# qwang-sj/qwen3-asr.cpp

Hardware: AMD Instinct MI355X
Metric: RTFx (audio-sec/wall-sec) + decode tokens/sec, Qwen3-ASR-0.6B f16 (higher is better)
Workload: dtype f16

## Files before the change

qwen3-asr.cpp_amd/csrc/attention.hip:

```cpp
#include <algorithm>
#include <type_traits>
#include <cstdlib>
#include <stdexcept>

#include "dev_common.h"
#include "fx_chain.h"
#include "fx_decode.h"
#include "kernels.h"

namespace qasr {

#define EKS 66
#define EVS 68

__global__ __launch_bounds__(256) void enc_attn_kernel(const float *__restrict__ qkv, const int *__restrict__ seg_start,
                                                       const int *__restrict__ seg_len, int D, uint16_t *__restrict__ out,
                                                       float *__restrict__ out32) {
    __shared__ __attribute__((aligned(16))) float Ks[64 * EKS];
    __shared__ __attribute__((aligned(16))) float Vs[64 * EVS];
    const int b = blockIdx.z, h = blockIdx.y;
    const int N = seg_len[b], r0 = seg_start[b];
    const int qblk = blockIdx.x * 64;
    if (qblk >= N) return;
    const int tid = threadIdx.x, lane = tid & 63, wid = tid >> 6;
// ... 1009 lines not shown
        if (c0 + 128 < nkv) kvc_issue(kc, vc, c0 + 128, kcap, want_v, A, a.kv_nt);
        kvc_step(a, qa, knew, vnew, c0 + 64, pos, B, st, sdst);
    }
    if constexpr (FX) {
        __syncthreads();
        mark(2);
        decode_attn_exact_body(a, 2 * g + (wid >> 1), b, wid & 1, fxs + (wid >> 1) * a.max_ctx);
        if (a.trace) __syncthreads();
        mark(3);
        stamp_end(a.stamp);
        return;
    }
    if (sdst) { stamp_end(a.stamp); return; }
#pragma unroll
    for (int e = 0; e < 8; e++) {
        st.o0[e] += __shfl_xor(st.o0[e], 16, 64);
        st.o0[e] += __shfl_xor(st.o0[e], 32, 64);
        st.o1[e] += __shfl_xor(st.o1[e], 16, 64);
        st.o1[e] += __shfl_xor(st.o1[e], 32, 64);
    }
    if (sub == 0) {
        *(floatx4 *)&wo[wid][0][dl] = floatx4{st.o0[0], st.o0[1], st.o0[2], st.o0[3]};
        *(floatx4 *)&wo[wid][0][dl + 4] = floatx4{st.o0[4], st.o0[5], st.o0[6], st.o0[7]};
        *(floatx4 *)&wo[wid][1][dl] = floatx4{st.o1[0], st.o1[1], st.o1[2], st.o1[3]};
        *(floatx4 *)&wo[wid][1][dl + 4] = floatx4{st.o1[4], st.o1[5], st.o1[6], st.o1[7]};
    }
    if (lane == 0) {
        wst[wid][0][0] = st.m0; wst[wid][0][1] = st.l0;
        wst[wid][1][0] = st.m1; wst[wid][1][1] = st.l1;
    }
    __syncthreads();
    const int hh = tid >> 7, d = tid & 127;
    float M = -INFINITY;
#pragma unroll
    for (int w = 0; w < 4; w++) M = fmaxf(M, wst[w][hh][0]);
    float L = 0.f, O = 0.f;
#pragma unroll
    for (int w = 0; w < 4; w++) {
        const float mw = wst[w][hh][0];
        const float f = mw == -INFINITY ? 0.f : expf(mw - M);
        L = fmaf(wst[w][hh][1], f, L);
        O = fmaf(wo[w][hh][d], f, O);
    }
    const float inv = L > 0.f ? 1.0f / L : 0.f;
    const float v = O * inv;
    const long e = (long)b * QD + (2 * g + hh) * 128 + d;
    if (a.outq) {
        float am = fabsf(v);
#pragma unroll
        for (int o = 1; o < 32; o <<= 1) am = fmaxf(am, __shfl_xor(am, o, 64));
        a.outq[e] = q8_quant(v, am);
        if ((d & 31) == 0) a.outd[e >> 5] = q8_scale(am);
    } else if (a.out32) a.out32[e] = v;
    else a.out[e] = f_to_u16(v);
    stamp_end(a.stamp);
}

int decode_stream_slots() {
    int nb = 0, dev = 0, cus = 0;
    if (hipGetDevice(&dev) != hipSuccess || hipDeviceGetAttribute(&cus, hipDeviceAttributeMultiprocessorCount, dev) != hipSuccess ||
        hipOccupancyMaxActiveBlocksPerMultiprocessor(&nb, reinterpret_cast<const void *>(decode_attn_seq_kernel<0>), 256, 0) !=
            hipSuccess)
        return 0;
    return nb * cus;
}

constexpr int ORPW = 1, OPROJ_ROWS = 4 * ORPW;
__device__ __forceinline__ void oproj1_body(const GemvArgs o, const DecodeAttnArgs a, int j) {
    constexpr int K = 2048, NT = 4;
    const int lane = threadIdx.x & 63, wid = threadIdx.x >> 6;
    const int row0 = j * OPROJ_ROWS + wid * ORPW;
    for (int i = 0; i < a.oproj_delay; i++) __builtin_amdgcn_s_sleep(8);
    half8 wv[ORPW][NT];
#pragma unroll
    for (int r = 0; r < ORPW; r++)
#pragma unroll
        for (int t = 0; t < NT; t++)
            wv[r][t] = __builtin_nontemporal_load((const half8 *)(o.W + (long)(row0 + r) * K + t * 512 + lane * 8));
    __shared__ int oready;
    if (threadIdx.x == 0) {
        int ok = 0;
        for (int it = 0; it < a.poll_limit; it++) {
            if (__hip_atomic_load(a.att_done + (j & 7) * 16, __ATOMIC_RELAXED, __HIP_MEMORY_SCOPE_AGENT) >=
                (unsigned)a.n_kv_head) {
                ok = 1;
                break;
            }
            __builtin_amdgcn_s_sleep(4);
        }
        if (a.fence) {
            __builtin_amdgcn_fence(__ATOMIC_ACQUIRE, "agent");
            asm volatile("s_waitcnt vmcnt(0)" ::: "memory");
        }
        if (!ok) __hip_atomic_fetch_or(a.err, (unsigned)DEVERR_O_WAIT, __ATOMIC_RELAXED, __HIP_MEMORY_SCOPE_AGENT);
        oready = ok;
    }
    __syncthreads();
    if (!oready) return;
    u32x4 xv[NT];
    ld_sc1_x4_4(o.xh + lane * 8, xv);
    float res[ORPW];
#pragma unroll
    for (int r = 0; r < ORPW; r++)
        res[r] = __uint_as_float(__hip_atomic_load((const uint32_t *)(o.res + row0 + r), __ATOMIC_RELAXED, __HIP_MEMORY_SCOPE_AGENT));
#pragma unroll
    for (int r = 0; r < ORPW; r++) {
        float acc = 0.f;
#pragma unroll
        for (int t = 0; t < NT; t++) {
            const half8 h = __builtin_bit_cast(half8, xv[t]);
#pragma unroll
            for (int e = 0; e < 8; e++) acc = fmaf((float)wv[r][t][e], (float)h[e], acc);
        }
        acc = wave_sum(acc);
        if (lane == 0) o.out_f32[row0 + r] = fadd_rn(acc, res[r]);
    }
}

__device__ __forceinline__ void ld_sc1_x4_8(const void *base, const uint32_t *off, u32x4 *v) {
    asm volatile(
        "global_load_dwordx4 %0, %8, %16 sc1\n\t"
        "global_load_dwordx4 %1, %9, %16 sc1\n\t"
        "global_load_dwordx4 %2, %10, %16 sc1\n\t"
        "global_load_dwordx4 %3, %11, %16 sc1\n\t"
        "global_load_dwordx4 %4, %12, %16 sc1\n\t"
        "global_load_dwordx4 %5, %13, %16 sc1\n\t"
        "global_load_dwordx4 %6, %14, %16 sc1\n\t"
        "global_load_dwordx4 %7, %15, %16 sc1\n\t"
        "s_waitcnt vmcnt(0)"
        : "=&v"(v[0]), "=&v"(v[1]), "=&v"(v[2]), "=&v"(v[3]), "=&v"(v[4]), "=&v"(v[5]), "=&v"(v[6]), "=&v"(v[7])
        : "v"(off[0]), "v"(off[1]), "v"(off[2]), "v"(off[3]), "v"(off[4]), "v"(off[5]), "v"(off[6]), "v"(off[7]), "s"(base)
        : "memory");
}
__host__ __device__ inline int fx_chain_wgs(int fx, int n_kv_head) { return fx ? n_kv_head : 0; }
struct alignas(16) ChainLds {
    float fsc[2][DX_KC / DX_B * FX_ST];
    uint16_t kmask[2][DX_KC / 16];
    float fwl[2];
};
__device__ __forceinline__ float fx1_gather_weights(const DecodeAttnArgs &a, const int g, const int n, ChainLds &C, const int trow) {
    auto &fsc = C.fsc;
    const int tid = threadIdx.x, lane = tid & 63, wid = tid >> 6;
    const int hh = wid >> 1, wu = __builtin_amdgcn_readfirstlane(wid & 1);
    auto mark = [&](int slot) {
        if (a.trace && tid == 0) a.trace[(long)trow * 8 + slot] = rt_now();
    };
    const uint32_t tag = gran_tag(a.pos[0], a.layer);
    const int np = (n + 1) >> 1;
    {
        const int ld = sgran_ld(a.max_ctx);
        const unsigned long long *gb = a.sgran + (long)(2 * g) * ld;
        uint32_t go[DX_KC / 256];
#pragma unroll
        for (int u = 0; u < DX_KC / 256; u++) {
            const int q = tid + 256 * (u >> 1);
            go[u] = q < np ? (uint32_t)(((u & 1) * ld + 2 * q) * 8) : 0u;
        }
        u32x4 gv[DX_KC / 256];
        bool ok = false;
        int it = 0;
        unsigned long long tis = 0;
        for (; it < a.poll_limit; it++) {
            if (a.trace) tis = rt_now();
            ld_sc1_x4_8(gb, go, gv);
            ok = true;
#pragma unroll
            for (int u = 0; u < DX_KC / 256; u++) {
                const int q = tid + 256 * (u >> 1);
                if (q < np) ok = ok && gv[u][1] == tag && (2 * q + 1 >= n || gv[u][3] == tag);
            }
            if (__syncthreads_and(ok)) break;
            __builtin_amdgcn_s_sleep(2);
        }
        if (a.trace && tid == 0) {
            a.trace[(4010L + g) * 8 + 5] = (unsigned long long)it + 1;
            a.trace[(4010L + g) * 8 + 6] = tis;
        }
        if (!ok && tid == 0) __hip_atomic_fetch_or(a.err, (unsigned)DEVERR_SCORE_WAIT, __ATOMIC_RELAXED, __HIP_MEMORY_SCOPE_AGENT);
#pragma unroll
        for (int u = 0; u < DX_KC / 256; u++) {
            const int q = tid + 256 * (u >> 1), j = 2 * q;
            if (q < np)
                *(float2 *)&fsc[u & 1][(j >> 5) * FX_ST + (j & 31)] = make_float2(__uint_as_float(gv[u][0]), __uint_as_float(gv[u][2]));
        }
    }
    __syncthreads();
    mark(2);
    auto &fwl = C.fwl;
    auto &kmask = C.kmask;
    float M, S;
    {
        float *row = fsc[hh] + lane * FX_ST;
        float sv[DX_B];
#pragma unroll
        for (int i = 0; i < DX_B; i += 4) {
            const floatx4 r = *(const floatx4 *)&row[i];
#pragma unroll
            for (int e = 0; e < 4; e++) sv[i + e] = lane * DX_B + i + e < n ? r[e] : -INFINITY;
        }
        float lm = -INFINITY, lh = -INFINITY;
#pragma unroll
        for (int i = 0; i < DX_B / 2; i++) lh = fmaxf(lh, sv[i]);
#pragma unroll
        for (int i = DX_B / 2; i < DX_B; i++) lm = fmaxf(lm, sv[i]);
        lm = fmaxf(lm, lh);
        const float inc = wave_scan_max(lm);
        const float Mp0 = dpp_ninf<0x138, 0xF>(inc);
        M = lane_f(inc, 63);
        float x[DX_B / 2];
        uint32_t kb = 0;
        auto half = [&](auto hc) {
            constexpr int H = decltype(hc)::value;
            float Mq = H ? fmaxf(Mp0, lh) : Mp0;
#pragma unroll
            for (int i = 0; i < DX_B / 2; i++) {
                const float sc = sv[H * (DX_B / 2) + i];
                const bool gt = sc > Mq;
                const float e = expf(gt ? Mq - sc : sc - Mq);
                x[i] = gt ? -e : (sc != -INFINITY ? e : 0.0f);
                kb |= (uint32_t)gt << i;
                Mq = fmaxf(Mq, sc);
            }
        };
        if (wu) half(std::integral_constant<int, 1>{});
        else half(std::integral_constant<int, 0>{});
        kmask[hh][2 * lane + wu] = (uint16_t)kb;
        __syncthreads();
        mark(6);
#pragma unroll
        for (int i = 0; i < DX_B / 2; i += 4) *(floatx4 *)&row[16 * wu + i] = floatx4{x[i], x[i + 1], x[i + 2], x[i + 3]};
        const int kl = n - 1;
        if (lane == (kl >> 5) && wu == ((kl >> 4) & 1)) {
            fwl[hh] = row[kl & 31];
            row[kl & 31] = 0.0f;
        }
        __syncthreads();
        mark(7);
        const float wl = fwl[hh];
        float Sl = 0.0f;
#pragma unroll
        for (int i = 0; i < DX_B; i += 4) {
            const floatx4 r = *(const floatx4 *)&row[i];
#pragma unroll
            for (int e = 0; e < 4; e++) Sl = __builtin_signbit(r[e]) ? fadd_rn(fmul_rn(Sl, -r[e]), 1.0f) : fadd_rn(fmul_rn(Sl, 1.0f), r[e]);
        }
        if (lane == (kl >> 5)) Sl = __builtin_signbit(wl) ? fadd_rn(fmul_rn(Sl, -wl), 1.0f) : fadd_rn(fmul_rn(Sl, 1.0f), wl);
        const float Ml = fmaxf(Mp0, lm);
        S = wave_sum(Ml == -INFINITY ? 0.0f : Sl * expf(Ml - M));
    }
    return S;
}
__device__ __forceinline__ void fx1_chain_body(const DecodeAttnArgs &a, const int g, ChainLds &C) {
    auto &fsc = C.fsc;
    const int tid = threadIdx.x, lane = tid & 63, wid = tid >> 6;
    const int hh = wid >> 1, wu = __builtin_amdgcn_readfirstlane(wid & 1);
    const int d = 64 * wu + lane, loff = 8 * lane;
    const uint16_t *vt = a.vt + (long)g * 128 * vt_ctx(a.max_ctx) + 64 * wu * 8;
    auto mark = [&](int slot) {
        if (a.trace && tid == 0) a.trace[(4000L + g) * 8 + slot] = rt_now();
    };
    mark(0);
    const int pos = a.pos[0], nkv = pos + 1;
    const uint32_t tag = gran_tag(pos, a.layer);
    const int QD = a.n_head * 128, KD = a.n_kv_head * 128;
    if (a.fx_vpf & 2) {
        typedef __attribute__((address_space(3))) void lds_void_c;
        typedef __attribute__((address_space(1))) void glb_void_c;
        lds_void_c *dst = (lds_void_c *)((float *)fsc + wid * 256);
        for (int kb = hh; kb * 8 < nkv; kb += 2)
            __builtin_amdgcn_global_load_lds((glb_void_c *)(vt + (long)kb * 1024 + loff), dst, 16, 0, 0);
    }
    const int n = nkv;
    const float S = fx1_gather_weights(a, g, n, C, 4000 + g);
    auto &fwl = C.fwl;
    auto &kmask = C.kmask;
    mark(3);
    uint16_t vnew = 0;
    {
        const unsigned long long *gp = a.gran + QD + KD + g * 128 + d;
        unsigned long long v = 0;
        bool ok = false;
        for (int it = 0; it < a.poll_limit; it++) {
            v = __hip_atomic_load(gp, __ATOMIC_RELAXED, __HIP_MEMORY_SCOPE_AGENT);
            ok = (uint32_t)(v >> 32) == tag;
            if (__all(ok)) break;
            __builtin_amdgcn_s_sleep(2);
        }
        if (!__all(ok) && lane == 0) __hip_atomic_fetch_or(a.err, (unsigned)DEVERR_QKV_WAIT, __ATOMIC_RELAXED, __HIP_MEMORY_SCOPE_AGENT);
        vnew = f_to_u16(__uint_as_float((uint32_t)v));
    }
    mark(1);
    const unsigned long long ck0 = a.trace ? clock64() : 0ull;
    f16 acc = 0;
    {
        const int nl = n - 1;
        u32x4 va[DX_Q / 8], vb[DX_Q / 8];
        floatx4 wa, wb;
        const int lastb = nl > 0 ? (nl - 1) >> 3 : 0;
        const int nfull = nl > 0 ? (lastb + 1) >> 3 : 0;
        constexpr uint32_t QB = DX_Q / 8 * 2048;
        const __amdgpu_buffer_rsrc_t vrs = __builtin_amdgcn_make_buffer_rsrc((void *)vt, (short)0, lastb * 2048 + 1024, 0x00020000);
        const uint32_t voff = 16 * lane;
        int jt = 0;
        fx_loadQ(va, vt, loff, 0, lastb);
        fx_w8(fsc[hh], 0, wa, wb);
        uint32_t bm = fx_buffer_bits(kmask[hh]);
        for (; jt + 2 * DX_Q < nfull * DX_Q; jt += 2 * DX_Q, bm >>= 2) {
            fx_loadQ_sb(vb, vrs, voff, (jt / DX_Q + 1) * QB);
            fx_step1_lds_b(va, jt, fsc[hh], kmask[hh], bm & 1u, acc, wa, wb);
            fx_loadQ_sb(va, vrs, voff, (jt / DX_Q + 2) * QB);
            fx_step1_lds_b(vb, jt + DX_Q, fsc[hh], kmask[hh], bm & 2u, acc, wa, wb);
        }
        for (int j0 = jt; j0 < nl; j0 += 2 * DX_Q, bm >>= 2) {
            fx_loadQ(vb, vt, loff, j0 + DX_Q, lastb);
            fx_step1_lds_b(va, j0, fsc[hh], kmask[hh], bm & 1u, acc, wa, wb);
            if (j0 + DX_Q >= nl) break;
            fx_loadQ(va, vt, loff, j0 + 2 * DX_Q, lastb);
            fx_step1_lds_b(vb, j0 + DX_Q, fsc[hh], kmask[hh], bm & 2u, acc, wa, wb);
        }
        acc = fx_key_slow(acc, vnew, fwl[hh]);
    }
    mark(4);
    if (a.trace && lane == 0) {
        a.trace[(4020L + g) * 8 + wid] = rt_now();
        a.trace[(4030L + g) * 8 + wid] = clock64() - ck0;
    }
    if (a.trace && tid == 0) {
        a.trace[(4010L + g) * 8 + 0] = ck0;
        a.trace[(4010L + g) * 8 + 1] = clock64();
        a.trace[(4010L + g) * 8 + 2] = (unsigned long long)n;
    }
    const float ov = (float)acc * (S == 0.0f ? 0.0f : 1.0f / S);
    const uint32_t h16 = f_to_u16(ov);
    const uint32_t hn = __shfl_xor(h16, 1, 64);
    uint16_t *out = a.out + (2 * g + hh) * 128 + d;
    if (a.att_done) {
        if ((lane & 1) == 0) __hip_atomic_store((uint32_t *)out, h16 | (hn << 16), __ATOMIC_RELAXED, __HIP_MEMORY_SCOPE_AGENT);
        asm volatile("s_waitcnt vmcnt(0)" ::: "memory");
        __syncthreads();
        if (a.fence && tid == 0) {
            __builtin_amdgcn_fence(__ATOMIC_RELEASE, "agent");
            asm volatile("s_waitcnt vmcnt(0)" ::: "memory");
        }
        if (a.fence) __syncthreads();
        if (tid < 8) __hip_atomic_fetch_add(a.att_done + tid * 16, 1u, __ATOMIC_RELAXED, __HIP_MEMORY_SCOPE_AGENT);
    } else {
        *out = (uint16_t)h16;
    }
    mark(5);
    if (a.trace && tid == 0) {
        unsigned nk = 0, ng = 0;
        for (int i = 0; i < DX_KC / 16; i++) {
            const unsigned m = kmask[0][i];
            nk += __builtin_popcount(m);
            ng += ((m & 0xffu) != 0) + ((m >> 8) != 0);
        }
        a.trace[(4010L + g) * 8 + 3] = nk;
        a.trace[(4010L + g) * 8 + 4] = ng;
    }
}

template <int SPL>
__global__ __launch_bounds__(256) void qkv_attn1_kernel(GemvArgs q, DecodeAttnArgs a, GemvArgs o) {
    constexpr int K = 1024, NT = 2, RPW = 2;
    constexpr size_t RLB = sizeof(SplitLds<SPL>) > sizeof(ChainLds) ? sizeof(SplitLds<SPL>) : sizeof(ChainLds);
    __shared__ __attribute__((aligned(16))) unsigned char role_lds[RLB];
    stamp_start(a.stamp);
    if (blockIdx.x >= 512) {
        const int j = blockIdx.x - 512, nsp = a.grid_splits, nat = nsp * a.n_kv_head;
        const int nfx = fx_chain_wgs(a.fx, a.n_kv_head);
        if (j >= nat + nfx) oproj1_body(o, a, j - nat - nfx);
        else if (j >= nat) fx1_chain_body(a, j - nat, *reinterpret_cast<ChainLds *>(role_lds));
        else decode_attn_body<SPL, true>(a, j / a.n_kv_head, j % a.n_kv_head, 0, nsp, *reinterpret_cast<SplitLds<SPL> *>(role_lds));
        stamp_end(a.stamp);
        return;
    }
    const int lane = threadIdx.x & 63, wid = threadIdx.x >> 6;
    const int grp = blockIdx.x >> 6, loc = blockIdx.x & 63;
    if (q.trace && threadIdx.x == 0) q.trace[blockIdx.x * 8] = rt_now();
    const int QD = a.n_head * 128, KD = a.n_kv_head * 128;
    const int rbase = loc < 32 ? grp * 256 + loc * 8 : loc < 48 ? QD + grp * 128 + (loc - 32) * 8 : QD + KD + grp * 128 + (loc - 48) * 8;
    const int row0 = rbase + wid * RPW;
    const uint32_t gtag = a.gran ? gran_tag(a.pos[0], a.layer) : 0u;
    half8 wv[RPW][NT];
#pragma unroll
    for (int r = 0; r < RPW; r++)
#pragma unroll
        for (int t = 0; t < NT; t++)
            wv[r][t] = __builtin_nontemporal_load((const half8 *)(q.W + (long)(row0 + r) * K + t * 512 + lane * 8));
    float xf[NT][8];
    if (q.embd_ids) {
        const uint16_t *er = q.embd + (long)q.embd_ids[0] * K;
#pragma unroll
        for (int t = 0; t < NT; t++) {
            const half8 h = *(const half8 *)(er + t * 512 + lane * 8);
#pragma unroll
            for (int e = 0; e < 8; e++) xf[t][e] = (float)h[e];
        }
        if (q.x_store && blockIdx.x == 0 && wid == 0)
#pragma unroll
            for (int t = 0; t < NT; t++)
#pragma unroll
                for (int e = 0; e < 8; e++)
                    __hip_atomic_store((uint32_t *)(q.x_store + t * 512 + lane * 8 + e), __float_as_uint(xf[t][e]), __ATOMIC_RELAXED,
                                       __HIP_MEMORY_SCOPE_AGENT);
    } else {
#pragma unroll
        for (int t = 0; t < NT; t++) {
            const float4 u = *(const float4 *)(q.x + t * 512 + lane * 8);
            const float4 v = *(const float4 *)(q.x + t * 512 + lane * 8 + 4);
            xf[t][0] = u.x; xf[t][1] = u.y; xf[t][2] = u.z; xf[t][3] = u.w;
            xf[t][4] = v.x; xf[t][5] = v.y; xf[t][6] = v.z; xf[t][7] = v.w;
        }
    }
    double ss = 0.0;
#pragma unroll
    for (int t = 0; t < NT; t++)
#pragma unroll
        for (int e = 0; e < 8; e++) ss += (double)(xf[t][e] * xf[t][e]);
    ss = wave_sum_d(ss);
    const float scale = 1.0f / sqrtf((float)(ss / K) + q.eps);
#pragma unroll
    for (int t = 0; t < NT; t++) {
        const float4 u = *(const float4 *)(q.norm_w + t * 512 + lane * 8);
        const float4 v = *(const float4 *)(q.norm_w + t * 512 + lane * 8 + 4);
        const float w[8] = {u.x, u.y, u.z, u.w, v.x, v.y, v.z, v.w};
#pragma unroll
        for (int e = 0; e < 8; e++) xf[t][e] = (float)f2h(fmul_rn(fmul_rn(xf[t][e], scale), w[e]));
    }
#pragma unroll
    for (int r = 0; r < RPW; r++) {
        float acc = 0.f;
#pragma unroll
        for (int t = 0; t < NT; t++)
#pragma unroll
            for (int e = 0; e < 8; e++) acc = fmaf((float)wv[r][t][e], xf[t][e], acc);
        acc = wave_sum(acc);
        if (a.gran) {
            if (lane == 0)
                __hip_atomic_store(a.gran + row0 + r, ((unsigned long long)gtag << 32) | __float_as_uint(acc), __ATOMIC_RELAXED,
                                   __HIP_MEMORY_SCOPE_AGENT);
        } else if (lane == 0) {
            __hip_atomic_store((uint32_t *)(q.out_f32 + row0 + r), __float_as_uint(acc), __ATOMIC_RELAXED, __HIP_MEMORY_SCOPE_AGENT);
        }
    }
    if (a.gran) {
        if (q.trace && threadIdx.x == 0) q.trace[blockIdx.x * 8 + 1] = rt_now();
        stamp_end(a.stamp);
        return;
    }
    asm volatile("s_waitcnt vmcnt(0)" ::: "memory");
    __syncthreads();
    if (a.fence && threadIdx.x == 0) {
        __builtin_amdgcn_fence(__ATOMIC_RELEASE, "agent");
        asm volatile("s_waitcnt vmcnt(0)" ::: "memory");
    }
    if (a.fence) __syncthreads();
    if (threadIdx.x < 8)
        __hip_atomic_fetch_add(a.qcnt + (grp * 8 + threadIdx.x) * 16, 1u, __ATOMIC_RELAXED, __HIP_MEMORY_SCOPE_AGENT);
    if (q.trace && threadIdx.x == 0) q.trace[blockIdx.x * 8 + 1] = rt_now();
    stamp_end(a.stamp);
}

static int split1(int spl1, int grid_splits) { return spl1 == 64 || spl1 == 128 ? spl1 : grid_splits >= 30 ? 128 : 64; }

int launch_qkv_attention1(const GemvArgs &q, const DecodeAttnArgs &a, const GemvArgs *o, const FuseCfg &cfg, hipStream_t s, bool dry) {
    if (!cfg.qkv || !cfg.err || a.B != 1 || !a.qcnt || q.M != 1 || q.K != 1024 || q.Wd || !q.norm_w || q.xh || q.bias || q.res ||
        a.out32 || a.outq || q.N != a.n_head * 128 + 2 * a.n_kv_head * 128 || a.n_head != 2 * a.n_kv_head || a.n_kv_head * 64 != 512)
        return 0;
    const int spl1 = split1(cfg.spl1, a.grid_splits);
    const int ns = (a.grid_splits * DSPLIT + spl1 - 1) / spl1;
    const bool with_o = cfg.o && o && a.att_done && o->M == 1 && o->K == 2048 && o->N == 1024 && o->xh && o->res &&
                        !o->Wd && !o->bias && !o->norm_w && o->xh == a.out;
    if (a.fx && (!a.gran || !a.sgran || ns * spl1 > DX_KC)) return 0;
    const int nfx = fx_chain_wgs(a.fx, a.n_kv_head);
    const int slots = spl1 == 128 ? cfg.slots_qkv128 : cfg.slots_qkv64;
    const int o_blocks = 1024 / OPROJ_ROWS;
    const bool fit_o = 512 + ns * a.n_kv_head + nfx + o_blocks <= slots;
    if (512 + ns * a.n_kv_head + nfx > slots) return 0;
    const bool with_o2 = with_o && fit_o;
    if (dry) return with_o2 ? 2 : 1;
    const dim3 grid(512 + ns * a.n_kv_head + nfx + (with_o2 ? o_blocks : 0));
    DecodeAttnArgs ad = a;
    ad.fuse_delay = cfg.qkv_delay;
    ad.oproj_delay = cfg.o_delay;
    ad.poll_limit = cfg.poll_limit;
    ad.fence = cfg.fence;
    ad.err = cfg.err;
    ad.grid_splits = ns;
    ad.fx_vpf = cfg.fx_vpf;
    if (!with_o2) ad.att_done = nullptr;
    const GemvArgs qa = q;
    const GemvArgs oa = with_o2 ? *o : GemvArgs{};
    if (spl1 == 128) hipLaunchKernelGGL(qkv_attn1_kernel<128>, grid, dim3(256), 0, s, qa, ad, oa);
    else hipLaunchKernelGGL(qkv_attn1_kernel<DSPLIT>, grid, dim3(256), 0, s, qa, ad, oa);
    return with_o2 ? 2 : 1;
}

void launch_decode_attention(const DecodeAttnArgs &a, hipStream_t s) {
    if (a.B <= 0) return;
    if (a.B <= 8) {
        if (split1(a.spl1, a.grid_splits) == 128) {
            const int g2 = (a.grid_splits * DSPLIT + 127) / 128;
            hipLaunchKernelGGL(decode_attn_kernel<128>, dim3(g2, a.n_kv_head, a.B), dim3(256), 0, s, a);
        } else {
            hipLaunchKernelGGL(decode_attn_kernel<DSPLIT>, dim3(a.grid_splits, a.n_kv_head, a.B), dim3(256), 0, s, a);
        }
    } else if (a.stream_blocks > 0 && a.n_head == 2 * a.n_kv_head && a.n_kv_head * a.B >= a.stream_blocks / 2) {
        hipLaunchKernelGGL(decode_attn_seq_kernel<0>, dim3(a.n_kv_head, a.B), dim3(256), 0, s, a);
    } else {
        if (a.spl_batch == 128) {
            const int g2 = (a.grid_splits * DSPLIT + 127) / 128;
            hipLaunchKernelGGL(decode_attn_kernel<128>, dim3(g2, a.n_kv_head, a.B), dim3(256), 0, s, a);
        } else {
            const int g4 = (a.grid_splits * DSPLIT + 255) / 256;
            hipLaunchKernelGGL(decode_attn_kernel<256>, dim3(g4, a.n_kv_head, a.B), dim3(256), 0, s, a);
        }
    }
}

bool launch_decode_attention_exact_seq(const DecodeAttnArgs &a, hipStream_t s) {
    const size_t lds = (size_t)2 * a.max_ctx * sizeof(float);
    if (!a.fx_seq || a.B <= 8 || a.stream_blocks <= 0 || a.n_head != 2 * a.n_kv_head || a.n_kv_head * a.B < a.stream_blocks / 2 ||
        lds > 32768)
        return false;
    hipLaunchKernelGGL(decode_attn_seq_kernel<1>, dim3(a.n_kv_head, a.B), dim3(256), lds, s, a);
    return true;
}

int fused_slots_ffn();

void fused_slots(FuseCfg &cfg) {
    auto slots_of = [](const void *kernel) {
        int nb = 0, dev = 0, cus = 0;
        if (hipGetDevice(&dev) != hipSuccess || hipDeviceGetAttribute(&cus, hipDeviceAttributeMultiprocessorCount, dev) != hipSuccess ||
            hipOccupancyMaxActiveBlocksPerMultiprocessor(&nb, kernel, 256, 0) != hipSuccess)
            return 0;
        return nb * cus;
    };
    cfg.slots_qkv64 = slots_of(reinterpret_cast<const void *>(qkv_attn1_kernel<DSPLIT>));
    cfg.slots_qkv128 = slots_of(reinterpret_cast<const void *>(qkv_attn1_kernel<128>));
    cfg.slots_ffn = fused_slots_ffn();
    cfg.slots_stream = decode_stream_slots();
}

int decode_split_len() { return DSPLIT; }
int decode_max_splits() { return 256; }

}
```

qwen3-asr.cpp_amd/csrc/fx_chain.h:

```cpp
#pragma once
#include "dev_common.h"

namespace qasr {

#define DX_B 32
#define DX_Q 64
#define DX_KC (64 * DX_B)

__device__ __forceinline__ f16 fx_cvt(float f) {
    f16 h;
    asm("v_cvt_f16_f32 %0, %1" : "=v"(h) : "v"(f));
    return h;
}
__device__ __forceinline__ f16 fx_mad1(f16 acc, uint16_t v, float vs) {
    return fx_cvt(fmaf((float)__builtin_bit_cast(f16, v), vs, (float)acc));
}

template <int CTRL, int ROWS>
__device__ __forceinline__ float dpp_ninf(float v) {
    return __builtin_bit_cast(float, __builtin_amdgcn_update_dpp(__builtin_bit_cast(int, -INFINITY), __builtin_bit_cast(int, v),
                                                                 CTRL, ROWS, 0xF, false));
}
__device__ __forceinline__ float wave_scan_max(float x) {
    x = fmaxf(x, dpp_ninf<0x111, 0xF>(x));
// ... 81 lines not shown
    const float *p = ws + (k >> 5) * FX_ST + (k & 31);
    wa = *(const floatx4 *)p;
    wb = *(const floatx4 *)(p + 4);
}
__device__ __forceinline__ void fx_step1_lds(const u32x4 *v, int j0, const float *ws, unsigned long long flags, f16 &acc,
                                             floatx4 &wa, floatx4 &wb) {
    if (__builtin_expect(((flags >> (j0 / DX_B)) & 3ull) != 0, 0)) {
#pragma unroll
        for (int g8 = 0; g8 < DX_Q / 8; g8++) {
            floatx4 na, nb;
            fx_w8(ws, j0 + 8 * g8 + 8, na, nb);
            fx8_slow(acc, v[g8], wa, wb);
            wa = na;
            wb = nb;
        }
    } else {
#pragma unroll
        for (int g8 = 0; g8 < DX_Q / 8; g8++) {
            floatx4 na, nb;
            fx_w8(ws, j0 + 8 * g8 + 8, na, nb);
            fx8_fast(acc, v[g8], wa, wb);
            wa = na;
            wb = nb;
        }
    }
}

__device__ __forceinline__ void fx_step1_lds_m(const u32x4 *v, int j0, const float *ws, unsigned long long m64, f16 &acc,
                                               floatx4 &wa, floatx4 &wb) {
    if (__builtin_expect(m64 != 0ull, 0)) {
#pragma unroll
        for (int g8 = 0; g8 < DX_Q / 8; g8++) {
            floatx4 na, nb;
            fx_w8(ws, j0 + 8 * g8 + 8, na, nb);
            if (((m64 >> (8 * g8)) & 0xffull) != 0) fx8_slow(acc, v[g8], wa, wb);
            else fx8_fast(acc, v[g8], wa, wb);
            wa = na;
            wb = nb;
        }
    } else {
#pragma unroll
        for (int g8 = 0; g8 < DX_Q / 8; g8++) {
            floatx4 na, nb;
            fx_w8(ws, j0 + 8 * g8 + 8, na, nb);
            fx8_fast(acc, v[g8], wa, wb);
            wa = na;
            wb = nb;
        }
    }
}
__device__ __forceinline__ unsigned long long fx_mask64(const uint16_t *km, int j0) {
    const uint2 m = *(const uint2 *)(km + j0 / 16);
    return ((unsigned long long)(uint32_t)__builtin_amdgcn_readfirstlane((int)m.y) << 32) |
           (uint32_t)__builtin_amdgcn_readfirstlane((int)m.x);
}

__device__ __forceinline__ void fx_step1_lds_b(const u32x4 *v, int j0, const float *ws, const uint16_t *km, bool hit, f16 &acc,
                                               floatx4 &wa, floatx4 &wb) {
    uint32_t fast = !hit;
    asm volatile("" : "+s"(fast));
    if (__builtin_expect(hit, 0)) {
        const unsigned long long m64 = fx_mask64(km, j0);
#pragma unroll
        for (int g8 = 0; g8 < DX_Q / 8; g8++) {
            floatx4 na, nb;
            fx_w8(ws, j0 + 8 * g8 + 8, na, nb);
            if (((m64 >> (8 * g8)) & 0xffull) != 0) fx8_slow(acc, v[g8], wa, wb);
            else fx8_fast(acc, v[g8], wa, wb);
            wa = na;
            wb = nb;
        }
    }
    if (__builtin_expect(fast != 0u, 1)) {
#pragma unroll
        for (int g8 = 0; g8 < DX_Q / 8; g8++) {
            floatx4 na, nb;
            fx_w8(ws, j0 + 8 * g8 + 8, na, nb);
            fx8_fast(acc, v[g8], wa, wb);
            wa = na;
            wb = nb;
        }
    }
}
__device__ __forceinline__ uint32_t fx_buffer_bits(const uint16_t *km) {
    static_assert(DX_KC / DX_Q == 32, "one bit a buffer in 32 bits");
    const uint2 m = *(const uint2 *)(km + 4 * (threadIdx.x & 31));
    return (uint32_t)__ballot((m.x | m.y) != 0u);
}

__device__ __forceinline__ void fx_loadQ_sb(u32x4 *v, __amdgpu_buffer_rsrc_t rs, uint32_t voff, uint32_t sb) {
#pragma unroll
    for (int i = 0; i < DX_Q / 8; i++)
        v[i] = __builtin_bit_cast(u32x4, __builtin_amdgcn_raw_buffer_load_b128(rs, voff + i * 2048, sb, 0));
}

__device__ __forceinline__ void fx_loadQ(u32x4 *v, const uint16_t *__restrict__ vt, int loff, int j0, int lastb = 1 << 28) {
#pragma unroll
    for (int i = 0; i < DX_Q / 8; i++) v[i] = *(const u32x4 *)(vt + (long)min(j0 / 8 + i, lastb) * 1024 + loff);
}

template <class Src>
__device__ __forceinline__ float fx_weights_reg(Src src, int n, float &M, float *w, unsigned long long &flags, float &wlast,
                                                uint32_t *kbits = nullptr) {
    const int lane = threadIdx.x & 63;
    float lm = -INFINITY;
#pragma unroll
    for (int i = 0; i < DX_B; i++) {
        const int j = lane * DX_B + i;
        w[i] = j < n ? src(j) : -INFINITY;
    }
#pragma unroll
    for (int i = 0; i < DX_B; i++) lm = fmaxf(lm, w[i]);
    const float inc = wave_scan_max(lm);
    float Mp = fmaxf(M, dpp_ninf<0x138, 0xF>(inc));
    const float Mn = fmaxf(M, lane_f(inc, 63));
    bool nm = false;
    uint32_t kb = 0;
#pragma unroll
    for (int i = 0; i < DX_B; i++) {
        const float s = w[i];
        const bool gt = s > Mp;
        const float e = expf(gt ? Mp - s : s - Mp);
        w[i] = gt ? -e : (s != -INFINITY ? e : 0.0f);
        Mp = fmaxf(Mp, s);
        nm = nm || gt;
        kb |= (uint32_t)gt << i;
    }
    if (kbits) *kbits = kb;
    float Sl = 0.0f, wl = 0.0f;
#pragma unroll
    for (int i = 0; i < DX_B; i++) {
        const float x = w[i];
        Sl = __builtin_signbit(x) ? fadd_rn(fmul_rn(Sl, -x), 1.0f) : fadd_rn(fmul_rn(Sl, 1.0f), x);
        if (lane * DX_B + i == n - 1) wl = x;
    }
    const float S = wave_sum(Mp == -INFINITY ? 0.0f : Sl * expf(Mp - Mn));
    flags = __ballot(nm || (lane + 1) * DX_B > n);
    wlast = lane_f(wl, (n - 1) / DX_B);
    M = Mn;
    return S;
}

}
```

Before: 278.3.

## Split fx chain per query head and pipeline score gathering with V accumulation

The fused chain attention now launches one workgroup per query head instead of per KV head. Inside each workgroup, two waves gather scores in 256-key chunks, compute softmax weights and key masks, and publish per-chunk progress flags in LDS. The other two waves stream V and accumulate as soon as each chunk is ready, rather than waiting for the whole score pass behind barriers. This overlaps score gathering with V reads and doubles chain parallelism. The cost is more workgroups competing for slots, more LDS, and spin-polling on LDS progress flags.

Result: faster. 296.5 (median of 6 runs) (+6.5%).

```diff
diff --git a/qwen3-asr.cpp_amd/csrc/attention.hip b/qwen3-asr.cpp_amd/csrc/attention.hip
--- a/qwen3-asr.cpp_amd/csrc/attention.hip
+++ b/qwen3-asr.cpp_amd/csrc/attention.hip
@@ -1115,7 +1115,7 @@
         int ok = 0;
         for (int it = 0; it < a.poll_limit; it++) {
             if (__hip_atomic_load(a.att_done + (j & 7) * 16, __ATOMIC_RELAXED, __HIP_MEMORY_SCOPE_AGENT) >=
-                (unsigned)a.n_kv_head) {
+                (unsigned)(a.fx ? a.n_head : a.n_kv_head)) {
                 ok = 1;
                 break;
             }
@@ -1150,226 +1150,240 @@
     }
 }
 
-__device__ __forceinline__ void ld_sc1_x4_8(const void *base, const uint32_t *off, u32x4 *v) {
-    asm volatile(
-        "global_load_dwordx4 %0, %8, %16 sc1\n\t"
-        "global_load_dwordx4 %1, %9, %16 sc1\n\t"
-        "global_load_dwordx4 %2, %10, %16 sc1\n\t"
-        "global_load_dwordx4 %3, %11, %16 sc1\n\t"
-        "global_load_dwordx4 %4, %12, %16 sc1\n\t"
-        "global_load_dwordx4 %5, %13, %16 sc1\n\t"
-        "global_load_dwordx4 %6, %14, %16 sc1\n\t"
-        "global_load_dwordx4 %7, %15, %16 sc1\n\t"
-        "s_waitcnt vmcnt(0)"
-        : "=&v"(v[0]), "=&v"(v[1]), "=&v"(v[2]), "=&v"(v[3]), "=&v"(v[4]), "=&v"(v[5]), "=&v"(v[6]), "=&v"(v[7])
-        : "v"(off[0]), "v"(off[1]), "v"(off[2]), "v"(off[3]), "v"(off[4]), "v"(off[5]), "v"(off[6]), "v"(off[7]), "s"(base)
-        : "memory");
-}
-__host__ __device__ inline int fx_chain_wgs(int fx, int n_kv_head) { return fx ? n_kv_head : 0; }
+__host__ __device__ inline int fx_chain_wgs(int fx, int n_head) { return fx ? n_head : 0; }
 struct alignas(16) ChainLds {
-    float fsc[2][DX_KC / DX_B * FX_ST];
-    uint16_t kmask[2][DX_KC / 16];
-    float fwl[2];
+    float fsc[DX_KC / DX_B * FX_ST];
+    uint16_t kmask[DX_KC / 16];
+    float gmax[DX_KC / DX_B];
+    uint32_t prog[DX_KC / FX_PC + 1];
+    float fwl, S;
+    float vpf[4][256];
 };
-__device__ __forceinline__ float fx1_gather_weights(const DecodeAttnArgs &a, const int g, const int n, ChainLds &C, const int trow) {
-    auto &fsc = C.fsc;
-    const int tid = threadIdx.x, lane = tid & 63, wid = tid >> 6;
-    const int hh = wid >> 1, wu = __builtin_amdgcn_readfirstlane(wid & 1);
-    auto mark = [&](int slot) {
-        if (a.trace && tid == 0) a.trace[(long)trow * 8 + slot] = rt_now();
-    };
+constexpr uint32_t FX_PUB = 0x8080u;
+__device__ __forceinline__ void fx1_gather_weights(const DecodeAttnArgs &a, const int head, const int n, ChainLds &C, const int p,
+                                                   unsigned long long *tr) {
+    const int lane = threadIdx.x & 63;
     const uint32_t tag = gran_tag(a.pos[0], a.layer);
-    const int np = (n + 1) >> 1;
+    const unsigned long long *gb = a.sgran + (long)head * sgran_ld(a.max_ctx);
+    unsigned char *pb = (unsigned char *)C.prog;
+    const int nch = (n + FX_PC - 1) / FX_PC, kl = n - 1;
+    float M = -INFINITY;
+    unsigned long long npoll = 0;
+    for (int ch = 0; ch < nch; ch++) {
+        const int k0 = ch * FX_PC + 4 * lane;
+        const unsigned long long *gp = gb + (k0 < n ? k0 : 0);
+        unsigned long long gv[4];
+        bool ok = false;
+        for (int it = 0; it < a.poll_limit; it++) {
+#pragma unroll
+            for (int e = 0; e < 4; e++) gv[e] = __hip_atomic_load(gp + e, __ATOMIC_RELAXED, __HIP_MEMORY_SCOPE_AGENT);
+            ok = true;
+#pragma unroll
+            for (int e = 0; e < 4; e++) ok = ok && (k0 + e >= n || (uint32_t)(gv[e] >> 32) == tag);
+            npoll++;
+            if (__all(ok)) break;
+            __builtin_amdgcn_s_sleep(2);
+        }
+        if (!__all(ok) && lane == 0) __hip_atomic_fetch_or(a.err, (unsigned)DEVERR_SCORE_WAIT, __ATOMIC_RELAXED, __HIP_MEMORY_SCOPE_AGENT);
+        float sv[4];
+#pragma unroll
+        for (int e = 0; e < 4; e++) sv[e] = k0 + e < n ? __uint_as_float((uint32_t)gv[e]) : -INFINITY;
+        const float lh = fmaxf(sv[0], sv[1]);
+        const float lm = fmaxf(lh, fmaxf(sv[2], sv[3]));
+        const float inc = wave_scan_max(lm);
+        const float Mp0 = fmaxf(M, dpp_ninf<0x138, 0xF>(inc));
+        const float Mi = fmaxf(M, inc);
+        M = fmaxf(M, lane_f(inc, 63));
+        uint32_t kb = 0;
+        {
+            float Mq = Mp0;
+#pragma unroll
+            for (int e = 0; e < 4; e++) {
+                kb |= (uint32_t)(sv[e] > Mq) << e;
+                Mq = fmaxf(Mq, sv[e]);
+            }
+        }
+        float x0, x1;
+        fx_weights2(p ? fmaxf(Mp0, lh) : Mp0, p ? sv[2] : sv[0], p ? sv[3] : sv[1], x0, x1);
+        const int k = k0 + 2 * p;
+        if (k == kl) { C.fwl = x0; x0 = 0.0f; }
+        if (k + 1 == kl) { C.fwl = x1; x1 = 0.0f; }
+        *(float2 *)&C.fsc[(k >> 5) * FX_ST + (k & 31)] = make_float2(x0, x1);
+        uint32_t m16 = kb << (4 * (lane & 3));
+        m16 |= __shfl_xor(m16, 1, 64);
+        m16 |= __shfl_xor(m16, 2, 64);
+        const uint32_t bits = fx_chunk_bits(kb);
+        if (p == 0) {
+            if ((lane & 3) == 0) C.kmask[ch * (FX_PC / 16) + (lane >> 2)] = (uint16_t)m16;
+            if ((lane & 7) == 7) C.gmax[ch * (FX_PC / DX_B) + (lane >> 3)] = Mi;
+        }
+        __builtin_amdgcn_fence(__ATOMIC_RELEASE, "workgroup");
+        if (lane == 0) __hip_atomic_store(pb + 4 * ch + p, (unsigned char)(0x80u | bits), __ATOMIC_RELAXED, __HIP_MEMORY_SCOPE_WORKGROUP);
+        if (tr && p == 0 && lane == 0 && (ch == 0 || ch == nch - 1)) {
+            if (ch == 0) tr[2] = rt_now();
+            if (ch == nch - 1) tr[3] = rt_now();
+        }
+    }
+    if (p != 0) return;
     {
-        const int ld = sgran_ld(a.max_ctx);
-        const unsigned long long *gb = a.sgran + (long)(2 * g) * ld;
-        uint32_t go[DX_KC / 256];
-#pragma unroll
-        for (int u = 0; u < DX_KC / 256; u++) {
-            const int q = tid + 256 * (u >> 1);
-            go[u] = q < np ? (uint32_t)(((u & 1) * ld + 2 * q) * 8) : 0u;
-        }
-        u32x4 gv[DX_KC / 256];
-        bool ok = false;
-        int it = 0;
-        unsigned long long tis = 0;
-        for (; it < a.poll_limit; it++) {
-            if (a.trace) tis = rt_now();
-            ld_sc1_x4_8(gb, go, gv);
-            ok = true;
-#pragma unroll
-            for (int u = 0; u < DX_KC / 256; u++) {
-                const int q = tid + 256 * (u >> 1);
-                if (q < np) ok = ok && gv[u][1] == tag && (2 * q + 1 >= n || gv[u][3] == tag);
-            }
-            if (__syncthreads_and(ok)) break;
-            __builtin_amdgcn_s_sleep(2);
-        }
-        if (a.trace && tid == 0) {
-            a.trace[(4010L + g) * 8 + 5] = (unsigned long long)it + 1;
-            a.trace[(4010L + g) * 8 + 6] = tis;
-        }
-        if (!ok && tid == 0) __hip_atomic_fetch_or(a.err, (unsigned)DEVERR_SCORE_WAIT, __ATOMIC_RELAXED, __HIP_MEMORY_SCOPE_AGENT);
-#pragma unroll
-        for (int u = 0; u < DX_KC / 256; u++) {
-            const int q = tid + 256 * (u >> 1), j = 2 * q;
-            if (q < np)
-                *(float2 *)&fsc[u & 1][(j >> 5) * FX_ST + (j & 31)] = make_float2(__uint_as_float(gv[u][0]), __uint_as_float(gv[u][2]));
-        }
-    }
-    __syncthreads();
-    mark(2);
-    auto &fwl = C.fwl;
-    auto &kmask = C.kmask;
-    float M, S;
-    {
-        float *row = fsc[hh] + lane * FX_ST;
-        float sv[DX_B];
+        uint32_t w = 0;
+        for (int it = 0; it < a.poll_limit; it++) {
+            w = __hip_atomic_load(pb + 4 * (nch - 1) + 1, __ATOMIC_RELAXED, __HIP_MEMORY_SCOPE_WORKGROUP);
+            if (w & 0x80u) break;
+            __builtin_amdgcn_s_sleep(1);
+        }
+        if (!(w & 0x80u) && lane == 0) __hip_atomic_fetch_or(a.err, (unsigned)DEVERR_SCORE_WAIT, __ATOMIC_RELAXED, __HIP_MEMORY_SCOPE_AGENT);
+        __builtin_amdgcn_fence(__ATOMIC_ACQUIRE, "workgroup");
+    }
+    float term = 0.0f;
+    if (lane * DX_B < nch * FX_PC) {
+        const float *row = C.fsc + lane * FX_ST;
+        const float wl = C.fwl;
+        float Sl = 0.0f;
 #pragma unroll
         for (int i = 0; i < DX_B; i += 4) {
             const floatx4 r = *(const floatx4 *)&row[i];
 #pragma unroll
-            for (int e = 0; e < 4; e++) sv[i + e] = lane * DX_B + i + e < n ? r[e] : -INFINITY;
-        }
-        float lm = -INFINITY, lh = -INFINITY;
-#pragma unroll
-        for (int i = 0; i < DX_B / 2; i++) lh = fmaxf(lh, sv[i]);
-#pragma unroll
-        for (int i = DX_B / 2; i < DX_B; i++) lm = fmaxf(lm, sv[i]);
-        lm = fmaxf(lm, lh);
-        const float inc = wave_scan_max(lm);
-        const float Mp0 = dpp_ninf<0x138, 0xF>(inc);
-        M = lane_f(inc, 63);
-        float x[DX_B / 2];
-        uint32_t kb = 0;
-        auto half = [&](auto hc) {
-            constexpr int H = decltype(hc)::value;
-            float Mq = H ? fmaxf(Mp0, lh) : Mp0;
-#pragma unroll
-            for (int i = 0; i < DX_B / 2; i++) {
-                const float sc = sv[H * (DX_B / 2) + i];
-                const bool gt = sc > Mq;
-                const float e = expf(gt ? Mq - sc : sc - Mq);
-                x[i] = gt ? -e : (sc != -INFINITY ? e : 0.0f);
-                kb |= (uint32_t)gt << i;
-                Mq = fmaxf(Mq, sc);
-            }
-        };
-        if (wu) half(std::integral_constant<int, 1>{});
-        else half(std::integral_constant<int, 0>{});
-        kmask[hh][2 * lane + wu] = (uint16_t)kb;
-        __syncthreads();
-        mark(6);
-#pragma unroll
-        for (int i = 0; i < DX_B / 2; i += 4) *(floatx4 *)&row[16 * wu + i] = floatx4{x[i], x[i + 1], x[i + 2], x[i + 3]};
-        const int kl = n - 1;
-        if (lane == (kl >> 5) && wu == ((kl >> 4) & 1)) {
-            fwl[hh] = row[kl & 31];
-            row[kl & 31] = 0.0f;
-        }
-        __syncthreads();
-        mark(7);
-        const float wl = fwl[hh];
-        float Sl = 0.0f;
-#pragma unroll
-        for (int i = 0; i < DX_B; i += 4) {
-            const floatx4 r = *(const floatx4 *)&row[i];
-#pragma unroll
             for (int e = 0; e < 4; e++) Sl = __builtin_signbit(r[e]) ? fadd_rn(fmul_rn(Sl, -r[e]), 1.0f) : fadd_rn(fmul_rn(Sl, 1.0f), r[e]);
         }
         if (lane == (kl >> 5)) Sl = __builtin_signbit(wl) ? fadd_rn(fmul_rn(Sl, -wl), 1.0f) : fadd_rn(fmul_rn(Sl, 1.0f), wl);
-        const float Ml = fmaxf(Mp0, lm);
-        S = wave_sum(Ml == -INFINITY ? 0.0f : Sl * expf(Ml - M));
-    }
-    return S;
-}
-__device__ __forceinline__ void fx1_chain_body(const DecodeAttnArgs &a, const int g, ChainLds &C) {
-    auto &fsc = C.fsc;
-    const int tid = threadIdx.x, lane = tid & 63, wid = tid >> 6;
-    const int hh = wid >> 1, wu = __builtin_amdgcn_readfirstlane(wid & 1);
+        const float Ml = C.gmax[lane];
+        term = Ml == -INFINITY ? 0.0f : Sl * expf(Ml - M);
+    }
+    const float S = wave_sum(term);
+    if (lane == 0) C.S = S;
+    __builtin_amdgcn_fence(__ATOMIC_RELEASE, "workgroup");
+    if (lane == 0) __hip_atomic_store(&C.prog[DX_KC / FX_PC], FX_PUB, __ATOMIC_RELAXED, __HIP_MEMORY_SCOPE_WORKGROUP);
+    if (tr && lane == 0) {
+        tr[6] = rt_now();
+        tr[7] = npoll;
+    }
+}
+__device__ __forceinline__ uint32_t fx1_progress(const DecodeAttnArgs &a, ChainLds &C, const int i) {
+    const uint32_t *pw = &C.prog[i];
+    uint32_t w = (uint32_t)__builtin_amdgcn_readfirstlane((int)__hip_atomic_load(pw, __ATOMIC_RELAXED, __HIP_MEMORY_SCOPE_WORKGROUP));
+    if (__builtin_expect((w & FX_PUB) != FX_PUB, 0)) {
+        for (int it = 0; it < a.poll_limit; it++) {
+            __builtin_amdgcn_s_sleep(1);
+            w = (uint32_t)__builtin_amdgcn_readfirstlane((int)__hip_atomic_load(pw, __ATOMIC_RELAXED, __HIP_MEMORY_SCOPE_WORKGROUP));
+            if ((w & FX_PUB) == FX_PUB) break;
+        }
+        if ((w & FX_PUB) != FX_PUB && (threadIdx.x & 63) == 0)
+            __hip_atomic_fetch_or(a.err, (unsigned)DEVERR_SCORE_WAIT, __ATOMIC_RELAXED, __HIP_MEMORY_SCOPE_AGENT);
+    }
+    __builtin_amdgcn_fence(__ATOMIC_ACQUIRE, "workgroup");
+    return w;
+}
+__device__ __forceinline__ void fx1_chain_body(const DecodeAttnArgs &a, const int c, ChainLds &C) {
+    const int tid = threadIdx.x, lane = tid & 63, wid = __builtin_amdgcn_readfirstlane(tid >> 6);
+    const int g = c % a.n_kv_head, hh = c / a.n_kv_head, head = 2 * g + hh;
+    const int wu = wid & 1;
     const int d = 64 * wu + lane, loff = 8 * lane;
     const uint16_t *vt = a.vt + (long)g * 128 * vt_ctx(a.max_ctx) + 64 * wu * 8;
+    unsigned long long *tr = a.trace ? a.trace + (4000L + c) * 8 : nullptr;
     auto mark = [&](int slot) {
-        if (a.trace && tid == 0) a.trace[(4000L + g) * 8 + slot] = rt_now();
+        if (tr && tid == 0) tr[slot] = rt_now();
     };
     mark(0);
-    const int pos = a.pos[0], nkv = pos + 1;
-    const uint32_t tag = gran_tag(pos, a.layer);
-    const int QD = a.n_head * 128, KD = a.n_kv_head * 128;
+    const int pos = a.pos[0], n = pos + 1;
+    if (tid <= DX_KC / FX_PC) C.prog[tid] = 0u;
     if (a.fx_vpf & 2) {
         typedef __attribute__((address_space(3))) void lds_void_c;
         typedef __attribute__((address_space(1))) void glb_void_c;
-        lds_void_c *dst = (lds_void_c *)((float *)fsc + wid * 256);
-        for (int kb = hh; kb * 8 < nkv; kb += 2)
+        lds_void_c *dst = (lds_void_c *)C.vpf[wid];
+        for (int kb = wid >> 1; kb * 8 < n; kb += 2)
             __builtin_amdgcn_global_load_lds((glb_void_c *)(vt + (long)kb * 1024 + loff), dst, 16, 0, 0);
     }
-    const int n = nkv;
-    const float S = fx1_gather_weights(a, g, n, C, 4000 + g);
-    auto &fwl = C.fwl;
-    auto &kmask = C.kmask;
-    mark(3);
-    uint16_t vnew = 0;
-    {
-        const unsigned long long *gp = a.gran + QD + KD + g * 128 + d;
-        unsigned long long v = 0;
-        bool ok = false;
-        for (int it = 0; it < a.poll_limit; it++) {
-            v = __hip_atomic_load(gp, __ATOMIC_RELAXED, __HIP_MEMORY_SCOPE_AGENT);
-            ok = (uint32_t)(v >> 32) == tag;
-            if (__all(ok)) break;
-            __builtin_amdgcn_s_sleep(2);
-        }
-        if (!__all(ok) && lane == 0) __hip_atomic_fetch_or(a.err, (unsigned)DEVERR_QKV_WAIT, __ATOMIC_RELAXED, __HIP_MEMORY_SCOPE_AGENT);
-        vnew = f_to_u16(__uint_as_float((uint32_t)v));
-    }
-    mark(1);
-    const unsigned long long ck0 = a.trace ? clock64() : 0ull;
-    f16 acc = 0;
-    {
+    __syncthreads();
+    if (wid >= 2) {
+        fx1_gather_weights(a, head, n, C, wid - 2, tr);
+    } else {
+        const uint32_t tag = gran_tag(pos, a.layer);
+        const int QD = a.n_head * 128, KD = a.n_kv_head * 128;
+        const float *fsc = C.fsc;
+        const uint16_t *kmask = C.kmask;
         const int nl = n - 1;
-        u32x4 va[DX_Q / 8], vb[DX_Q / 8];
-        floatx4 wa, wb;
-        const int lastb = nl > 0 ? (nl - 1) >> 3 : 0;
-        const int nfull = nl > 0 ? (lastb + 1) >> 3 : 0;
-        constexpr uint32_t QB = DX_Q / 8 * 2048;
-        const __amdgpu_buffer_rsrc_t vrs = __builtin_amdgcn_make_buffer_rsrc((void *)vt, (short)0, lastb * 2048 + 1024, 0x00020000);
-        const uint32_t voff = 16 * lane;
-        int jt = 0;
-        fx_loadQ(va, vt, loff, 0, lastb);
-        fx_w8(fsc[hh], 0, wa, wb);
-        uint32_t bm = fx_buffer_bits(kmask[hh]);
-        for (; jt + 2 * DX_Q < nfull * DX_Q; jt += 2 * DX_Q, bm >>= 2) {
-            fx_loadQ_sb(vb, vrs, voff, (jt / DX_Q + 1) * QB);
-            fx_step1_lds_b(va, jt, fsc[hh], kmask[hh], bm & 1u, acc, wa, wb);
-            fx_loadQ_sb(va, vrs, voff, (jt / DX_Q + 2) * QB);
-            fx_step1_lds_b(vb, jt + DX_Q, fsc[hh], kmask[hh], bm & 2u, acc, wa, wb);
-        }
-        for (int j0 = jt; j0 < nl; j0 += 2 * DX_Q, bm >>= 2) {
-            fx_loadQ(vb, vt, loff, j0 + DX_Q, lastb);
-            fx_step1_lds_b(va, j0, fsc[hh], kmask[hh], bm & 1u, acc, wa, wb);
-            if (j0 + DX_Q >= nl) break;
-            fx_loadQ(va, vt, loff, j0 + 2 * DX_Q, lastb);
-            fx_step1_lds_b(vb, j0 + DX_Q, fsc[hh], kmask[hh], bm & 2u, acc, wa, wb);
-        }
-        acc = fx_key_slow(acc, vnew, fwl[hh]);
-    }
-    mark(4);
-    if (a.trace && lane == 0) {
-        a.trace[(4020L + g) * 8 + wid] = rt_now();
-        a.trace[(4030L + g) * 8 + wid] = clock64() - ck0;
-    }
-    if (a.trace && tid == 0) {
-        a.trace[(4010L + g) * 8 + 0] = ck0;
-        a.trace[(4010L + g) * 8 + 1] = clock64();
-        a.trace[(4010L + g) * 8 + 2] = (unsigned long long)n;
-    }
-    const float ov = (float)acc * (S == 0.0f ? 0.0f : 1.0f / S);
-    const uint32_t h16 = f_to_u16(ov);
-    const uint32_t hn = __shfl_xor(h16, 1, 64);
-    uint16_t *out = a.out + (2 * g + hh) * 128 + d;
+        if (a.trace && nl > 0) {
+            (void)fx1_progress(a, C, 0);
+            mark(1);
+        }
+        const unsigned long long ck0 = a.trace ? clock64() : 0ull;
+        f16 acc = 0;
+        {
+            u32x4 va[DX_Q / 8], vb[DX_Q / 8];
+            floatx4 wa, wb;
+            const int lastb = nl > 0 ? (nl - 1) >> 3 : 0;
+            const int nfull = nl > 0 ? (lastb + 1) >> 3 : 0;
+            constexpr uint32_t QB = DX_Q / 8 * 2048;
+            const __amdgpu_buffer_rsrc_t vrs = __builtin_amdgcn_make_buffer_rsrc((void *)vt, (short)0, lastb * 2048 + 1024, 0x00020000);
+            const uint32_t voff = 16 * lane;
+            int jt = 0;
+            fx_loadQ(va, vt, loff, 0, lastb);
+            uint32_t bm = 0;
+            const float *wrow = fsc;
+            const uint16_t *krow = kmask;
+            for (; jt + 2 * DX_Q < nfull * DX_Q; jt += 2 * DX_Q, bm >>= 2, wrow += 2 * DX_Q / DX_B * FX_ST, krow += 2 * DX_Q / 16) {
+                fx_loadQ_sb(vb, vrs, voff, (jt / DX_Q + 1) * QB);
+                if ((jt & (FX_PC - 1)) == 0) {
+                    bm = fx1_progress(a, C, jt / FX_PC);
+                    fx_w8(wrow, 0, wa, wb);
+                }
+                fx_step1_lds_b(va, 0, wrow, krow, bm & 1u, acc, wa, wb);
+                fx_loadQ_sb(va, vrs, voff, (jt / DX_Q + 2) * QB);
+                fx_step1_lds_b(vb, DX_Q, wrow, krow, bm & 2u, acc, wa, wb);
+            }
+            for (int j0 = jt; j0 < nl; j0 += 2 * DX_Q, bm >>= 2) {
+                fx_loadQ(vb, vt, loff, j0 + DX_Q, lastb);
+                if ((j0 & (FX_PC - 1)) == 0) {
+                    bm = fx1_progress(a, C, j0 / FX_PC);
+                    fx_w8(fsc, j0, wa, wb);
+                }
+                fx_step1_lds_b(va, j0, fsc, kmask, bm & 1u, acc, wa, wb);
+                if (j0 + DX_Q >= nl) break;
+                fx_loadQ(va, vt, loff, j0 + 2 * DX_Q, lastb);
+                fx_step1_lds_b(vb, j0 + DX_Q, fsc, kmask, bm & 2u, acc, wa, wb);
+            }
+        }
+        const unsigned long long ck1 = a.trace ? clock64() : 0ull;
+        uint16_t vnew = 0;
+        {
+            const unsigned long long *gp = a.gran + QD + KD + g * 128 + d;
+            unsigned long long v = 0;
+            bool ok = false;
+            for (int it = 0; it < a.poll_limit; it++) {
+                v = __hip_atomic_load(gp, __ATOMIC_RELAXED, __HIP_MEMORY_SCOPE_AGENT);
+                ok = (uint32_t)(v >> 32) == tag;
+                if (__all(ok)) break;
+                __builtin_amdgcn_s_sleep(2);
+            }
+            if (!__all(ok) && lane == 0) __hip_atomic_fetch_or(a.err, (unsigned)DEVERR_QKV_WAIT, __ATOMIC_RELAXED, __HIP_MEMORY_SCOPE_AGENT);
+            vnew = f_to_u16(__uint_as_float((uint32_t)v));
+        }
+        (void)fx1_progress(a, C, DX_KC / FX_PC);
+        const float S = C.S;
+        acc = fx_key_slow(acc, vnew, C.fwl);
+        mark(4);
+        if (a.trace && lane == 0) {
+            a.trace[(4080L + c) * 8 + wid] = rt_now();
+            a.trace[(4080L + c) * 8 + 2 + wid] = ck1 - ck0;
+        }
+        if (a.trace && tid == 0) {
+            a.trace[(4040L + c) * 8 + 0] = ck0;
+            a.trace[(4040L + c) * 8 + 1] = ck1;
+            a.trace[(4040L + c) * 8 + 2] = (unsigned long long)n;
+        }
+        const float ov = (float)acc * (S == 0.0f ? 0.0f : 1.0f / S);
+        const uint32_t h16 = f_to_u16(ov);
+        const uint32_t hn = __shfl_xor(h16, 1, 64);
+        uint16_t *out = a.out + head * 128 + d;
+        if (a.att_done) {
+            if ((lane & 1) == 0) __hip_atomic_store((uint32_t *)out, h16 | (hn << 16), __ATOMIC_RELAXED, __HIP_MEMORY_SCOPE_AGENT);
+            asm volatile("s_waitcnt vmcnt(0)" ::: "memory");
+        } else {
+            *out = (uint16_t)h16;
+        }
+    }
     if (a.att_done) {
-        if ((lane & 1) == 0) __hip_atomic_store((uint32_t *)out, h16 | (hn << 16), __ATOMIC_RELAXED, __HIP_MEMORY_SCOPE_AGENT);
-        asm volatile("s_waitcnt vmcnt(0)" ::: "memory");
         __syncthreads();
         if (a.fence && tid == 0) {
             __builtin_amdgcn_fence(__ATOMIC_RELEASE, "agent");
@@ -1377,19 +1391,17 @@
         }
         if (a.fence) __syncthreads();
         if (tid < 8) __hip_atomic_fetch_add(a.att_done + tid * 16, 1u, __ATOMIC_RELAXED, __HIP_MEMORY_SCOPE_AGENT);
-    } else {
-        *out = (uint16_t)h16;
     }
     mark(5);
     if (a.trace && tid == 0) {
         unsigned nk = 0, ng = 0;
-        for (int i = 0; i < DX_KC / 16; i++) {
-            const unsigned m = kmask[0][i];
+        for (int i = 0; i < (n + FX_PC - 1) / FX_PC * (FX_PC / 16); i++) {
+            const unsigned m = C.kmask[i];
             nk += __builtin_popcount(m);
             ng += ((m & 0xffu) != 0) + ((m >> 8) != 0);
         }
-        a.trace[(4010L + g) * 8 + 3] = nk;
-        a.trace[(4010L + g) * 8 + 4] = ng;
+        a.trace[(4040L + c) * 8 + 3] = nk;
+        a.trace[(4040L + c) * 8 + 4] = ng;
     }
 }
 
@@ -1401,7 +1413,7 @@
     stamp_start(a.stamp);
     if (blockIdx.x >= 512) {
         const int j = blockIdx.x - 512, nsp = a.grid_splits, nat = nsp * a.n_kv_head;
-        const int nfx = fx_chain_wgs(a.fx, a.n_kv_head);
+        const int nfx = fx_chain_wgs(a.fx, a.n_head);
         if (j >= nat + nfx) oproj1_body(o, a, j - nat - nfx);
         else if (j >= nat) fx1_chain_body(a, j - nat, *reinterpret_cast<ChainLds *>(role_lds));
         else decode_attn_body<SPL, true>(a, j / a.n_kv_head, j % a.n_kv_head, 0, nsp, *reinterpret_cast<SplitLds<SPL> *>(role_lds));
@@ -1506,7 +1518,7 @@
     const bool with_o = cfg.o && o && a.att_done && o->M == 1 && o->K == 2048 && o->N == 1024 && o->xh && o->res &&
                         !o->Wd && !o->bias && !o->norm_w && o->xh == a.out;
     if (a.fx && (!a.gran || !a.sgran || ns * spl1 > DX_KC)) return 0;
-    const int nfx = fx_chain_wgs(a.fx, a.n_kv_head);
+    const int nfx = fx_chain_wgs(a.fx, a.n_head);
     const int slots = spl1 == 128 ? cfg.slots_qkv128 : cfg.slots_qkv64;
     const int o_blocks = 1024 / OPROJ_ROWS;
     const bool fit_o = 512 + ns * a.n_kv_head + nfx + o_blocks <= slots;
diff --git a/qwen3-asr.cpp_amd/csrc/fx_chain.h b/qwen3-asr.cpp_amd/csrc/fx_chain.h
--- a/qwen3-asr.cpp_amd/csrc/fx_chain.h
+++ b/qwen3-asr.cpp_amd/csrc/fx_chain.h
@@ -187,10 +187,21 @@
         }
     }
 }
-__device__ __forceinline__ uint32_t fx_buffer_bits(const uint16_t *km) {
-    static_assert(DX_KC / DX_Q == 32, "one bit a buffer in 32 bits");
-    const uint2 m = *(const uint2 *)(km + 4 * (threadIdx.x & 31));
-    return (uint32_t)__ballot((m.x | m.y) != 0u);
+#define FX_PC 256
+__device__ __forceinline__ uint32_t fx_chunk_bits(uint32_t kb4) {
+    static_assert(FX_PC == 4 * 64 && FX_PC / DX_Q == 4, "four keys a lane, four buffers a chunk");
+    const unsigned long long bl = __ballot(kb4 != 0u);
+    return (uint32_t)((bl & 0xffffull) != 0) | (uint32_t)(((bl >> 16) & 0xffffull) != 0) << 1 |
+           (uint32_t)(((bl >> 32) & 0xffffull) != 0) << 2 | (uint32_t)((bl >> 48) != 0) << 3;
+}
+__device__ __forceinline__ void fx_weights2(float Mq, float s0, float s1, float &x0, float &x1) {
+    const bool g0 = s0 > Mq;
+    const float e0 = expf(g0 ? Mq - s0 : s0 - Mq);
+    x0 = g0 ? -e0 : (s0 != -INFINITY ? e0 : 0.0f);
+    Mq = fmaxf(Mq, s0);
+    const bool g1 = s1 > Mq;
+    const float e1 = expf(g1 ? Mq - s1 : s1 - Mq);
+    x1 = g1 ? -e1 : (s1 != -INFINITY ? e1 : 0.0f);
 }
 
 __device__ __forceinline__ void fx_loadQ_sb(u32x4 *v, __amdgpu_buffer_rsrc_t rs, uint32_t voff, uint32_t sb) {
```
